# thrill/thrill

Measured on AMD Instinct MI355X. Metric: TeraSort keys/sec (100-byte recs), higher is better.
Workload: dtype u8; 1 GPU; terasort_10GiB_100B; records=107374182, record_bytes=100, seed=0x7421, parallelism=dp1

## Files before the change

### include/thrill_amd.h

```cpp
#ifndef THRILL_AMD_H
#define THRILL_AMD_H

#include <stdint.h>

#ifdef __cplusplus
extern "C" {
#endif

typedef struct t9_context t9_context;

int t9_create(t9_context** out, int device, int rank, int world, void* comm);
int t9_destroy(t9_context* ctx);
const char* t9_version(void);

int t9_comm_id_size(void);
int t9_comm_id(void* out_id);
int t9_comm_init(t9_context* ctx, const void* id);

int t9_gen_u64(t9_context* ctx, uint64_t* d_out, uint64_t index0, uint64_t n,
               uint64_t seed, void* stream);
int t9_gen_records(t9_context* ctx, uint8_t* d_out, uint64_t index0,
                   uint64_t n, uint64_t seed, void* stream);


// ... 18 lines not shown
                          uint32_t rec_size, int le, uint64_t* d_keys,
                          uint32_t* d_idx, uint32_t* d_hist, void* stream);

int t9_gather_records(t9_context* ctx, const uint8_t* d_recs,
                      const uint32_t* d_idx, uint64_t n, uint32_t rec_size,
                      uint8_t* d_out, void* stream);

uint64_t t9_sort_records_workspace(uint64_t n, uint32_t rec_size);
int t9_sort_records(t9_context* ctx, const uint8_t* d_in, uint8_t* d_out,
                    uint64_t n, uint32_t rec_size, uint32_t key_len,
                    void* d_workspace, void* stream);

int t9_sort_records_keyle(t9_context* ctx, const uint8_t* d_in,
                          uint8_t* d_out, uint64_t n, uint32_t rec_size,
                          void* d_workspace, void* stream);

int t9_sort_last_schedule(const t9_context* ctx);

int t9_sort_last_tiecount(const t9_context* ctx);

int t9_sort_last_fused(const t9_context* ctx);

int t9_sort_last_packed(const t9_context* ctx);


int t9_classify_u64(t9_context* ctx, const uint64_t* d_keys, uint64_t n,
                    uint64_t gidx0, const uint64_t* d_spl_keys,
                    const uint64_t* d_spl_idx, uint32_t p,
                    uint32_t* d_bucket, uint64_t* d_counts, void* stream);

int t9_classify_rec(t9_context* ctx, const uint8_t* d_recs,
                    const uint64_t* d_k64, uint64_t n, uint64_t gidx0,
                    const uint8_t* d_spl_recs, const uint64_t* d_spl_k64,
                    const uint64_t* d_spl_idx, uint32_t p, uint32_t rec_size,
                    uint32_t* d_bucket, uint64_t* d_counts, void* stream);

uint64_t t9_partition_idx_workspace(uint64_t n);
int t9_partition_idx(t9_context* ctx, const uint32_t* d_bucket, uint64_t n,
                     uint32_t p, uint32_t* d_perm, uint64_t* d_offsets,
                     void* d_workspace, void* stream);

int t9_alltoall(t9_context* ctx, const void* d_send,
                const uint64_t* send_counts, const uint64_t* send_displs,
                void* d_recv, const uint64_t* recv_counts,
                const uint64_t* recv_displs, uint64_t elem_size,
                void* stream);
// ... 148 lines not shown
```

### thrill_amd/csrc/t9_api.cpp

```cpp

#include "t9_common.h"

#include <rccl/rccl.h>

#include <cstdlib>
#include <cstring>
#include <new>

extern "C" {

const char* t9_version(void) { return "thrill_amd 0.1 (gfx950)"; }

int t9_create(t9_context** out, int device, int rank, int world,
              void* comm) {
    if (!out || world < 1 || rank < 0 || rank >= world) return T9_EINVAL;
    HIP_TRY(hipSetDevice(device));
    t9_context* ctx = new (std::nothrow) t9_context;
    if (!ctx) return T9_ENOMEM;
    ctx->device = device;
    ctx->rank = rank;
    ctx->world = world;
    ctx->comm = comm;
    ctx->owns_comm = 0;
    ctx->ov_stream = nullptr;
    for (int i = 0; i <= T9_OVERLAP_MAXK; ++i) ctx->ov_ev[i] = nullptr;
    ctx->ov_ready = 0;
    ctx->last_schedule = 0;
    ctx->last_tiecount = 0;
    ctx->last_fused = 0;
    ctx->last_packed = 0;
    *out = ctx;
    return T9_OK;
}

int t9_destroy(t9_context* ctx) {
    if (ctx && ctx->comm && ctx->owns_comm)
        ncclCommDestroy((ncclComm_t)ctx->comm);
    if (ctx) {
        if (ctx->ov_stream) {
            (void)hipStreamSynchronize(ctx->ov_stream);
            (void)hipStreamDestroy(ctx->ov_stream);
        }
        for (int i = 0; i <= T9_OVERLAP_MAXK; ++i)
            if (ctx->ov_ev[i]) (void)hipEventDestroy(ctx->ov_ev[i]);
    }
    delete ctx;
    return T9_OK;
}

int t9i_overlap_init(t9_context* ctx) {
    if (!ctx) return T9_EINVAL;
    if (ctx->ov_ready) return T9_OK;
    HIP_TRY(hipSetDevice(ctx->device));
// ... 2 lines not shown
                                         hipStreamNonBlocking));
    for (int i = 0; i <= T9_OVERLAP_MAXK; ++i)
        if (!ctx->ov_ev[i])
            HIP_TRY(hipEventCreateWithFlags(&ctx->ov_ev[i],
                                            hipEventDisableTiming));
    ctx->ov_ready = 1;
    return T9_OK;
}

int t9_sort_last_schedule(const t9_context* ctx) {
    return ctx ? ctx->last_schedule : T9_EINVAL;
}

int t9_sort_last_tiecount(const t9_context* ctx) {
    return ctx ? ctx->last_tiecount : T9_EINVAL;
}

int t9_sort_last_fused(const t9_context* ctx) {
    return ctx ? ctx->last_fused : T9_EINVAL;
}

int t9_sort_last_packed(const t9_context* ctx) {
    return ctx ? ctx->last_packed : T9_EINVAL;
}


int t9_comm_id_size(void) { return (int)sizeof(ncclUniqueId); }

int t9_comm_id(void* out_id) {
    if (!out_id) return T9_EINVAL;
    ncclResult_t rc = ncclGetUniqueId((ncclUniqueId*)out_id);
    if (rc != ncclSuccess) {
        fprintf(stderr, "t9_comm_id: %s\n", ncclGetErrorString(rc));
        return T9_EIO;
    }
    return T9_OK;
}

int t9_comm_init(t9_context* ctx, const void* id) {
    if (!ctx || !id) return T9_EINVAL;
    if (ctx->comm) return T9_EINVAL;
    HIP_TRY(hipSetDevice(ctx->device));
    ncclComm_t comm = nullptr;
    ncclResult_t rc = ncclCommInitRank(&comm, ctx->world,
                                       *(const ncclUniqueId*)id, ctx->rank);
    if (rc != ncclSuccess) {
// ... 68 lines not shown
```

### thrill_amd/csrc/t9_common.h

```cpp
#pragma once

#include <hip/hip_runtime.h>
#include <cstdint>
#include <cstdio>

#include "thrill_amd.h"

using u8 = uint8_t;
using u16 = uint16_t;
using u32 = uint32_t;
using u64 = uint64_t;

#define T9_WAVE 64

#define T9_OK 0
#define T9_EINVAL (-22)
#define T9_ENOMEM (-12)
#define T9_EIO (-5)
#define T9_ENOSYS (-38)

#define HIP_TRY(expr)                                                     \
    do {                                                                  \
        hipError_t _e = (expr);                                           \
        if (_e != hipSuccess) {                                           \
// ... 8 lines not shown
        hipError_t _e = hipGetLastError();                                \
        if (_e != hipSuccess) {                                           \
            fprintf(stderr, "t9: %s:%d: kernel launch failed: %s\n",      \
                    __FILE__, __LINE__, hipGetErrorString(_e));           \
            return T9_EIO;                                                \
        }                                                                 \
    } while (0)

#define T9_OVERLAP_MAXK 16

struct t9_context {
    int device;
    int rank;
    int world;
    void* comm;
    int owns_comm;
    hipStream_t ov_stream;
    hipEvent_t ov_ev[T9_OVERLAP_MAXK + 1];
    int ov_ready;
    int last_schedule;
    int last_tiecount;
    int last_fused;
    int last_packed;
};

#define T9_PK_IBITS 27
#define T9_PK_IMASK ((1u << T9_PK_IBITS) - 1u)

struct t9_overlap_req {
    const u8* recs;
    u8* out;
    u32 rec_words;
    u32 chunks;
    u32 fused;
    u32 keyle;
    u32 packed;
};

__host__ __device__ inline u64 t9_splitmix64_at(u64 seed, u64 ctr) {
    u64 z = seed + (ctr + 1) * 0x9E3779B97F4A7C15ull;
    z = (z ^ (z >> 30)) * 0xBF58476D1CE4E5B9ull;
    z = (z ^ (z >> 27)) * 0x94D049BB133111EBull;
    return z ^ (z >> 31);
}

__host__ __device__ inline u64 t9_hash128to64(u64 upper, u64 lower) {
    const u64 k = 0x9DDFEA08EB382D69ull;
    u64 a = (lower ^ upper) * k;
    a ^= (a >> 47);
    u64 b = (upper ^ a) * k;
    b ^= (b >> 47);
    b *= k;
    return b;
}

#define T9_MSB 0x8000000000000000ull

__host__ __device__ inline u64 t9_enc(u64 b, int op, int vtype) {
    if (op == T9_OP_SUM || vtype == T9_VAL_U64) return b;
// ... 28 lines not shown
```

### thrill_amd/csrc/t9_rank_scatter.h

```cpp
#pragma once
#include "t9_common.h"

template <int NDIG>
__device__ inline void t9_scan_onewave(u32* s_vals, u32 tid) {
    if (tid < 64) {
        const u32 lane = tid;
        u32 carry = 0;
        for (int c = 0; c < NDIG / 64; ++c) {
            const u32 v0 = s_vals[c * 64 + lane];
            u32 v = v0;
            for (int off = 1; off < 64; off <<= 1) {
                u32 y = __shfl_up(v, off);
                if (lane >= (u32)off) v += y;
            }
            const u32 total = __shfl(v, 63);
            s_vals[c * 64 + lane] = (v - v0) + carry;
            carry += total;
        }
    }
}

__device__ inline void t9_scan256_onewave(u32* s_vals, u32 tid) {
    if (tid < 64) {
        const u32 lane = tid;
// ... 162 lines not shown
            gpos[c] = s_goff[d] + (j - s_start[d]);
            out_keys[gpos[c]] = k;
        }
    }
    if (!HAS_VAL) return;
    __syncthreads();

#pragma unroll
    for (int g = 0; g < GROUPS; ++g) {
        const u32 i = wbase + g * 64 + lane;
        if (i < tn) {
            const u32 pos = (pos2[g >> 1] >> (16 * (g & 1))) & 0xffffu;
            if constexpr (LOAD_VAL) s_ovals[pos] = val[g];
            else s_ovals[pos] = (u32)(base + i);
        }
    }
    __syncthreads();
#pragma unroll
    for (int c = 0; c < GROUPS; ++c) {
        const u32 j = c * BLOCK + tid;
        if (j < tn) out_vals[gpos[c]] = s_ovals[j];
    }
}
```

### thrill_amd/csrc/t9_records.hip

```cpp

#include "t9_common.h"
#include "t9_rank_scatter.h"

#include <cstdlib>
#include <cstring>
#include <vector>
#include <algorithm>

extern "C" int t9i_sort_pairs_msb_unpacked_redo(u64*, u32*, u64, void*,
                                                void*, t9_overlap_req*,
                                                u32*);
extern "C" int t9i_count_tied(const u64* d_keys, u64 n, u32* d_ntied,
                              hipStream_t s);
extern "C" u64 t9_sort_pairs_workspace(u64 n);
extern "C" int t9_sort_pairs_u64_u32(t9_context*, u64*, u32*, u64, void*,
                                     void*);
extern "C" int t9i_sort_recs_msb(t9_context*, const u8*, u32, u64*, u32*,
                                 u64, void*, void*);
extern "C" u64 t9_partition_idx_workspace(u64 n);
extern "C" int t9_partition_idx(t9_context*, const u32*, u64, u32, u32*,
                                u64*, void*, void*);
extern "C" int t9i_sort_pairs_msb_ph(t9_context*, u64*, u32*, u64, void*,
                                     void*, int, t9_overlap_req*, u32*,
                                     int*);
// ... 783 lines not shown
        return T9_OK;
    }
    char* p = (char*)d_workspace;
    u64* d_keys = (u64*)p;
    p += t9_align256(n * 8);
    u32* d_idx = (u32*)p;
    p += t9_align256(n * 4);
    void* pair_ws = p;
    p += t9_sort_pairs_workspace(n);
    u32* d_ntied = (u32*)p;

    const char* algo = getenv("T9_SORT_ALGO");
    bool msb_dispatch = n >= (1ull << 22);
    if (algo && strcmp(algo, "lsd") == 0) msb_dispatch = false;
    if (algo && strcmp(algo, "msb") == 0) msb_dispatch = n >= (1ull << 14);
    const char* ehe = getenv("T9_EXTRACT_HIST");
    const u32 rw = rec_size / 4;
    const bool eh = !(ehe && ehe[0] == '0') && msb_dispatch &&
                    (rw == 25 || rw == 32);
    const char* fe = getenv("T9_FUSED_EXTRACT");
    bool fused = fe && atoi(fe) && n >= (1ull << 14) &&
                 (rec_size == 100 || rec_size == 128);
    int rc;
    t9_overlap_req ov = { nullptr, nullptr, 0, 0, 0, le ? 1u : 0u, 0 };
    int tie_counted = 0;
    if (ctx) {
        ctx->last_schedule = 0;
        ctx->last_tiecount = 0;
        ctx->last_fused = 0;
        ctx->last_packed = 0;
    }
    if (eh && !fused) {
        u32* hist = t9i_msb_pass1_hist(pair_ws, n);
        const u64 B = t9_ceil_div(n, 8192);
        const char* ie = getenv("T9_EXTRACT_IOTA");
        const bool widx = ie && ie[0] == '1';
        T9_PERF_WRAP(s, "extract",
                     launch_extract_hist_any(widx, rw, le, (u32)B, s, d_in,
                                             n, d_keys, d_idx, hist));
        T9_LAUNCH_CHECK();
        const char* gv = getenv("T9_GATHER_VARIANT");
        const bool may_overlap = rw == 25 && ctx && !(gv && atoi(gv) != 3);
        if (may_overlap) {
            ov.recs = d_in;
            ov.out = d_out;
            ov.rec_words = rw;
        }
        rc = t9i_sort_pairs_msb_ph(ctx, d_keys, d_idx, n, pair_ws, stream,
                                   widx ? 0 : 1, may_overlap ? &ov : nullptr,
                                   d_ntied, &tie_counted);
    }
    else if (fused && !le) {
        rc = t9i_sort_recs_msb(ctx, d_in, rec_size, d_keys, d_idx, n,
                               pair_ws, stream);
    }
    else {
        rc = le ? t9_extract_key64_le(ctx, d_in, n, rec_size, 0, d_keys,
                                      d_idx, stream)
                : t9_extract_key64(ctx, d_in, n, rec_size, 0, d_keys,
                                   d_idx, stream);
        if (rc) return rc;
        rc = t9_sort_pairs_u64_u32(ctx, d_keys, d_idx, n, pair_ws, stream);
    }
    if (rc) return rc;
    if (!tie_counted) {
        rc = t9i_count_tied(d_keys, n, d_ntied, s);
        if (rc) return rc;
    }
    if (ctx) ctx->last_tiecount = tie_counted;
    u32 ntied = 0;
    HIP_TRY(hipMemcpyAsync(&ntied, d_ntied, 4, hipMemcpyDeviceToHost, s));
    HIP_TRY(hipStreamSynchronize(s));
    if (ov.packed) {
        ctx->last_packed = ntied ? 2 : 1;
        if (ntied) {
            rc = t9i_sort_pairs_msb_unpacked_redo(d_keys, d_idx, n, pair_ws,
                                                  stream, &ov, d_ntied);
            if (rc) return rc;
            HIP_TRY(hipMemcpyAsync(&ntied, d_ntied, 4,
                                   hipMemcpyDeviceToHost, s));
            HIP_TRY(hipStreamSynchronize(s));
        }
    }
    if (ov.chunks) {
        ctx->last_schedule = (int)ov.chunks;
        if (!ntied) return T9_OK;
    }
    if (ov.fused) {
        ctx->last_fused = ntied ? 2 : 1;
        if (!ntied) return T9_OK;
    }

    if (ntied && rec_size > 8) {
        const u64 need = 6 * t9_align256(n * 4) +
                         2 * t9_align256(n * 8) +
                         t9_align256(3 * 8) + 256 +
                         t9_align256((n / T9_MAXSCAN_TILE + 2) * 4) + 256 +
                         t9_partition_idx_workspace(n);
        void* tmp_alloc = nullptr;
        char* q;
        if ((u64)n * rec_size >= need) {
            q = (char*)d_out;
        }
        else {
            HIP_TRY(hipMalloc(&tmp_alloc, need));
            q = (char*)tmp_alloc;
// ... 180 lines not shown
```

### thrill_amd/csrc/t9_sort_msb.hip

```cpp

#include "t9_common.h"
#include "t9_rank_scatter.h"
#include "t9_bitonic.h"

#include <cstdlib>
#include <vector>

#define T9_MSB_TILE 8192
#define T9_SUBMAX 4096
#define T9_MSB_MIN (1u << 22)

__global__ void k_colsum(const u32*, u64, u32*);
__global__ void k_chunkscan(u32*, u64, u32*);
__global__ void k_finaloffs(u32*, u64, const u32*, const u32*);
__global__ void k_grp_scan(u32*, u64, u64*);

extern "C" void t9i_launch_hist_seg9(u32, void*, const u64*, const u32*,
                                     const u32*, u32*);
extern "C" void t9i_launch_seg_scan9(u32, void*, u32*, const u32*,
                                     const u32*, const u32*, u32*, u32*);
extern "C" void t9i_launch_scatter_seg9(u32, int, void*, const u64*,
                                        const u32*, const u32*, const u32*,
                                        u64*, u32*, const u32*);
extern "C" void t9i_launch_scatter_seg9_packed(u32, void*, const u64*,
                                               const u32*, const u32*,
                                               const u32*, u64*, const u32*);
constexpr u64 NSUB9 = 256ull * 512;

static int pass2_bits() {
    const char* e = getenv("T9_PASS2_BITS");
    return (e && atoi(e) == 8) ? 8 : 9;
}

#define T9_L3_MIN 240000000ull

extern "C" int t9i_sort_pairs_lsd(t9_context*, u64*, u32*, u64, void*,
                                  void*);
extern "C" u64 t9i_sort_pairs_lsd_workspace(u64 n);
extern "C" int t9i_sort_keys_lsd(t9_context*, u64*, u64, void*, void*);


template <int RW>
__global__ __launch_bounds__(256) void k_hist_msb(
    const u64* __restrict__ keys, u64 n, u32 shift, u32* __restrict__ hist) {
    __shared__ u32 s_cnt[T9_RADIX];
    const u32 tid = threadIdx.x;
    const u64 base = (u64)blockIdx.x * T9_MSB_TILE;
    const u32 tn =
        (u32)((n - base < (u64)T9_MSB_TILE) ? (n - base) : (u64)T9_MSB_TILE);
// ... 908 lines not shown
#endif
#ifndef T9_FUSED_DEFAULT
#define T9_FUSED_DEFAULT 1
#endif

static bool t9i_fused_gather() {
    const char* e = getenv("T9_SORT_FUSED_GATHER");
    if (!e || e[0] == '\0') return T9_FUSED_DEFAULT != 0;
    return e[0] != '0';
}

static bool t9i_packed_ok(u64 n) {
    const char* e = getenv("T9_SORT_PACKED");
    if (e && e[0] == '0') return false;
    u32 bits = T9_PK_IBITS;
    const char* b = getenv("T9_SORT_PACKED_IDXBITS");
    if (b && b[0]) {
        const int v = atoi(b);
        if (v >= 1 && v < (int)T9_PK_IBITS) bits = (u32)v;
    }
    return n <= (1ull << bits);
}

static void t9i_launch_fused_wide(hipStream_t s, u64* d_keys, u32* d_vals,
                                  const u32* sub_start, const u32* sub_n,
                                  u32* tcount, const t9_overlap_req* ov) {
    hipLaunchKernelGGL(
        (k_wave16_sort_gather<T9_FUSED_D, T9_FUSED_TIES != 0>),
        dim3((u32)NSUB9), dim3(64), 0, s, d_keys, d_vals, sub_start, sub_n,
        tcount, (const u32*)ov->recs, (u32*)ov->out);
}

__global__ __launch_bounds__(64) void k_chunk_bounds(
    const u32* __restrict__ sub_start, u32 nsub, u32 K,
    const u32* __restrict__ info, u32* __restrict__ out) {
    const u32 c = threadIdx.x;
    if (c < 2) out[c] = info[c];
    if (c >= 1 && c < K)
        out[1 + c] = sub_start[(u64)c * nsub / K];
}

template <bool HAS_VAL, int RW = 0>
static int sort_msb_impl(t9_context* ctx, const u64* pass1_src,
                         u64* d_keys, u32* d_vals, u64 n,
                         void* d_workspace, void* stream,
                         bool pre_hist = false,
                         t9_overlap_req* ov = nullptr,
                         bool iota_vals = false,
                         u32* d_ntied = nullptr,
                         int* tie_counted = nullptr) {
    hipStream_t s = (hipStream_t)stream;
    MsbWs w = carve_msb((char*)d_workspace, n);

    {
        const u64 B = w.B1;
        const u64 Bc = t9_ceil_div(B, T9_SCAN_CHUNK);
        if (!pre_hist)
            T9_PERF_WRAP(s, "hist_pairs",
                         hipLaunchKernelGGL((k_hist_msb<RW>), dim3((u32)B),
                                            dim3(256), 0, s, pass1_src, n,
                                            56, w.hist));
        hipLaunchKernelGGL(k_colsum, dim3((u32)Bc), dim3(256), 0, s, w.hist,
                           B, w.chunkpart);
        hipLaunchKernelGGL(k_chunkscan, dim3(1), dim3(256), 0, s,
                           w.chunkpart, Bc, w.digit_base);
        hipLaunchKernelGGL(k_align_bases, dim3(1), dim3(256), 0, s,
                           w.digit_base, n, w.true_base, w.abase,
                           w.bucket_n);
        hipLaunchKernelGGL(k_finaloffs, dim3((u32)Bc), dim3(256), 0, s,
                           w.hist, B, w.chunkpart, w.abase);
        T9_PERF_WRAP(
            s, "pair_scatter",
            if (HAS_VAL && !RW && iota_vals)
                hipLaunchKernelGGL(
                    (k_scatter_wave512<T9_MSB_TILE, 1024, true, HAS_VAL, 0,
                                       true>),
                    dim3((u32)B), dim3(1024), 0, s, pass1_src, d_vals,
                    w.alt_k, w.alt_v, w.hist, n, 56);
            else
                hipLaunchKernelGGL(
                    (k_scatter_wave512<T9_MSB_TILE, 1024, true, HAS_VAL,
                                       RW>),
                    dim3((u32)B), dim3(1024), 0, s, pass1_src, d_vals,
                    w.alt_k, w.alt_v, w.hist, n, 56));
        T9_LAUNCH_CHECK();
    }

    {
        const char* l3x = getenv("T9_MSB_LEVELS");
        const bool blocked3 = (n >= T9_L3_MIN) ||
                              (l3x && atoi(l3x) == 3 && n >= (1ull << 14));
        if (pass2_bits() == 9 && !blocked3) {
            const u64 B2 = t9_ceil_div(n, T9_MSB_TILE) + 256;
            T9_PERF_WRAP(s, "hist_pairs",
                         t9i_launch_hist_seg9((u32)B2, stream, w.alt_k,
                                              w.abase, w.bucket_n,
                                              w.hist));
            t9i_launch_seg_scan9(256, stream, w.hist, w.abase, w.bucket_n,
                                 w.true_base, w.sub_start, w.sub_n);
            HIP_TRY(hipMemsetAsync(w.ovr, 0, 8, s));
            hipLaunchKernelGGL(k_subinfo, dim3((u32)(NSUB9 / 256)),
                               dim3(256), 0, s, w.sub_n, (u32)NSUB9,
                               T9_SUBMAX, NSUB, w.ovr, w.ovr + 2);
            const u32 K = (HAS_VAL && ov && ctx && !t9perf_on() &&
                           t9i_lds_wave16())
                              ? overlap_chunks() : 0;
            u32 info[2 + T9_OVERLAP_MAXK] = { 0, 0 };
            if (K) {
                hipLaunchKernelGGL(k_chunk_bounds, dim3(1), dim3(64), 0, s,
                                   w.sub_start, (u32)NSUB9, K, w.ovr,
                                   w.span);
                HIP_TRY(hipMemcpyAsync(info, w.span, (K + 1) * 4,
                                       hipMemcpyDeviceToHost, s));
            }
            else
                HIP_TRY(hipMemcpyAsync(info, w.ovr, 8,
                                       hipMemcpyDeviceToHost, s));
            HIP_TRY(hipStreamSynchronize(s));
            const u32 maxsub = info[0], novr9 = info[1];
            u32* tcount = nullptr;
            if constexpr (HAS_VAL) {
                if (d_ntied && novr9 == 0 &&
                    t9i_lds_wave16() && maxsub <= t9i_wave16_max()) {
                    tcount = d_ntied;
                    HIP_TRY(hipMemsetAsync(tcount, 0, 4, s));
                    if (tie_counted) *tie_counted = 1;
                }
            }
            bool fuse = false, packed = false;
            if constexpr (HAS_VAL) {
                fuse = tcount && ov && ctx && !t9perf_on() && ov->recs &&
                       ov->rec_words == 25 && overlap_chunks() == 0 &&
                       maxsub <= 1024 && t9i_fused_gather();
                packed = fuse && t9i_packed_ok(n);
            }
            if (packed)
                t9i_launch_scatter_seg9_packed((u32)B2, stream, w.alt_k,
                                               w.alt_v, w.abase, w.bucket_n,
                                               d_keys, w.hist);
            else
                T9_PERF_WRAP(s, "pair_scatter",
                             t9i_launch_scatter_seg9((u32)B2, HAS_VAL,
                                                     stream, w.alt_k,
                                                     w.alt_v, w.abase,
                                                     w.bucket_n, d_keys,
                                                     d_vals, w.hist));
            T9_LAUNCH_CHECK();
            if (K && tcount) {
                u64 bnd[T9_OVERLAP_MAXK + 1];
                bnd[0] = 0;
                bnd[K] = n;
                bool mono = true;
                for (u32 c = 1; c < K; ++c) {
                    bnd[c] = info[1 + c];
                    mono = mono && bnd[c] >= bnd[c - 1] && bnd[c] <= n;
                }
                if (mono) {
                    int rc = t9i_overlap_init(ctx);
                    if (rc) return rc;
// ... 19 lines not shown
                    }
                    HIP_TRY(hipEventRecord(ctx->ov_ev[T9_OVERLAP_MAXK], sb));
                    HIP_TRY(hipStreamWaitEvent(
                        s, ctx->ov_ev[T9_OVERLAP_MAXK], 0));
                    ov->chunks = done;
                    return T9_OK;
                }
            }
            if constexpr (HAS_VAL) {
                if (fuse) {
                    if (packed)
                        hipLaunchKernelGGL(
                            (k_wave16_sort_gather_packed<T9_FUSED_D>),
                            dim3((u32)NSUB9), dim3(64), 0, s, d_keys,
                            w.sub_start, w.sub_n, tcount,
                            (const u32*)ov->recs, (u32*)ov->out, ov->keyle,
                            (u32)(n - 1));
                    else
                        t9i_launch_fused_wide(s, d_keys, d_vals, w.sub_start,
                                              w.sub_n, tcount, ov);
                    T9_LAUNCH_CHECK();
                    ov->fused = 1;
                    ov->packed = packed ? 1 : 0;
                    return T9_OK;
                }
            }
            T9_PERF_WRAP(
                s, "lds_sort",
                if (t9i_lds_wave16() && maxsub <= t9i_wave16_max())
                    t9i_launch_wave16_sub<HAS_VAL>((u32)NSUB9, maxsub, s,
                                                   d_keys, d_vals,
                                                   w.sub_start, w.sub_n,
                                                   tcount);
                else if (t9i_lds_bitonic())
                    t9i_launch_bitonic_sub<HAS_VAL>((u32)NSUB9, maxsub, s,
                                                    d_keys, d_vals,
                                                    w.sub_start, w.sub_n);
                else if (maxsub <= 1024)
                    hipLaunchKernelGGL(
                        (k_lds_sort_sub<1024, 256, HAS_VAL>), dim3(NSUB9),
                        dim3(256), 0, s, d_keys, d_vals, w.sub_start,
                        w.sub_n);
                else if (maxsub <= 2048)
                    hipLaunchKernelGGL(
                        (k_lds_sort_sub<2048, 512, HAS_VAL>), dim3(NSUB9),
                        dim3(512), 0, s, d_keys, d_vals, w.sub_start,
// ... 322 lines not shown
```

### thrill_amd/csrc/t9_sort_msb9.hip

```cpp

#include "t9_common.h"
#include "t9_rank_scatter.h"

#include <cstdlib>
#include <vector>

#define T9_MSB_TILE 8192
#define NDIG9 512

__device__ inline u32 bucket_of9(const u32* s_abase, u32 pos) {
    u32 lo = 0, hi = 255;
    while (lo < hi) {
        u32 mid = (lo + hi + 1) >> 1;
        if (s_abase[mid] <= pos) lo = mid; else hi = mid - 1;
    }
    return lo;
}

__global__ __launch_bounds__(256) void k_hist_seg9(
    const u64* __restrict__ keys, const u32* __restrict__ abase,
    const u32* __restrict__ bucket_n, u32* __restrict__ hist) {
    __shared__ u32 s_cnt[NDIG9];
    __shared__ u32 s_abase[257];
    const u32 tid = threadIdx.x;
    s_abase[tid] = abase[tid];
    if (tid == 0) s_abase[256] = abase[256];
    s_cnt[tid] = 0;
    s_cnt[tid + 256] = 0;
    __syncthreads();
    const u64 tbase64 = (u64)blockIdx.x * T9_MSB_TILE;
    if (tbase64 < s_abase[256]) {
        const u32 tbase = (u32)tbase64;
        const u32 b = bucket_of9(s_abase, tbase);
        const u32 off = tbase - s_abase[b];
        const u32 tn = (bucket_n[b] > off)
                           ? ((bucket_n[b] - off < T9_MSB_TILE)
                                  ? bucket_n[b] - off
                                  : T9_MSB_TILE)
                           : 0;
        const u32 lane = tid & 63;
        for (u32 i0 = 0; i0 < (u32)T9_MSB_TILE; i0 += 256) {
            const u32 i = i0 + tid;
            const bool valid = i < tn;
            const u32 d =
                valid ? (u32)(keys[tbase + i] >> 47) & 511u : 0;
            t9_hist_ballot_add<9>(s_cnt, d, valid, lane);
        }
    }
    __syncthreads();
    hist[(u64)blockIdx.x * NDIG9 + tid] = s_cnt[tid];
    hist[(u64)blockIdx.x * NDIG9 + tid + 256] = s_cnt[tid + 256];
}

__global__ __launch_bounds__(256) void k_seg_scan9(
    u32* __restrict__ hist, const u32* __restrict__ abase,
    const u32* __restrict__ bucket_n, const u32* __restrict__ true_base,
    u32* __restrict__ sub_start, u32* __restrict__ sub_n) {
    const u32 b = blockIdx.x;
    const u32 tid = threadIdx.x;
    const u32 r0 = abase[b] / T9_MSB_TILE;
    const u32 rows = (bucket_n[b] + T9_MSB_TILE - 1) / T9_MSB_TILE;
    u32 tot0 = 0, tot1 = 0;
    for (u32 r = 0; r < rows; ++r) {
        tot0 += hist[(u64)(r0 + r) * NDIG9 + tid];
        tot1 += hist[(u64)(r0 + r) * NDIG9 + tid + 256];
    }
    __shared__ u32 sh[NDIG9];
    sh[tid] = tot0;
// ... 167 lines not shown
#pragma unroll
        for (int g = 0; g < GROUPS; ++g) {
            const u32 i = wbase + g * 64 + lane;
            if (i < tn)
                s_ovals[(pos2[g >> 1] >> (16 * (g & 1))) & 0xffffu] = val[g];
        }
        __builtin_amdgcn_sched_barrier(0);
    }
#pragma unroll
    for (int c = 0; c < GROUPS; ++c)
        if (c * 1024 + tid < tn) out_keys[gpos[c]] = k[c];
    if (!HAS_VAL) return;
    __syncthreads();
    {
        u32 v[GROUPS];
#pragma unroll
        for (int c = 0; c < GROUPS; ++c) v[c] = s_ovals[c * 1024 + tid];
#pragma unroll
        for (int c = 0; c < GROUPS; ++c)
            if (c * 1024 + tid < tn) out_vals[gpos[c]] = v[c];
    }
}

__global__ __launch_bounds__(1024, 8) void k_scatter_seg9_packed(
    const u64* __restrict__ in_keys, const u32* __restrict__ in_vals,
    const u32* __restrict__ abase, const u32* __restrict__ bucket_n,
    u64* __restrict__ out_comp, const u32* __restrict__ offs) {
    constexpr int TILE = T9_MSB_TILE;
    constexpr int NW = 16;
    constexpr int SUB = TILE / NW;
    constexpr int GROUPS = SUB / 64;
    __shared__ __align__(16) u8 s_raw[TILE * 8];
    u64* const s_ocomp = (u64*)s_raw;
    static_assert(SUB <= 65535 && TILE <= 65535, "u16 counts and offsets");
    static_assert(NW * 64 == 1024 && NDIG9 == 8 * 64,
                  "one thread per key column, waves 0..7 own the digits");
    __shared__ __align__(16) u16 s_wcnt[NW * NDIG9];
    u32* const s_wtot = (u32*)s_raw;
    u32* const s_delta = (u32*)s_wcnt;
    u8* const s_dig8 = (u8*)s_wcnt + NDIG9 * 4;
    u32* const s_hi = (u32*)((u8*)s_wcnt + NDIG9 * 4 + TILE);
    static_assert(NDIG9 * 4 + TILE + 4 <= NW * NDIG9 * 2,
                  "the overlays fit the count array");

    const u32 tid = threadIdx.x, wave = tid >> 6, lane = tid & 63;
    const u32 xper = gridDim.x >> 3, xrem = gridDim.x & 7;
    const u32 xcd = blockIdx.x & 7;
    const u32 tile = xcd * xper + (xcd < xrem ? xcd : xrem) +
                     (blockIdx.x >> 3);
    const u64 tbase64 = (u64)tile * TILE;
    if (tbase64 >= abase[256]) return;
    const u32 tbase = (u32)tbase64;

    const u32 wbase = wave * SUB;
    u64 key[GROUPS];
#pragma unroll
    for (int g = 0; g < GROUPS; ++g)
        key[g] = in_keys[tbase + wbase + g * 64 + lane];
    u32 val[GROUPS];
#pragma unroll
    for (int g = 0; g < GROUPS; ++g)
        val[g] = in_vals[tbase + wbase + g * 64 + lane];
    u32 ab[4], bnq[4];
#pragma unroll
    for (int q = 0; q < 4; ++q) {
        ab[q] = abase[q * 64 + lane];
        bnq[q] = bucket_n[q * 64 + lane];
    }
    u16* const wc = s_wcnt + wave * NDIG9;
    for (u32 t = lane; t < NDIG9; t += 64) wc[t] = 0;

    u32 nle = 0;
#pragma unroll
    for (int q = 0; q < 4; ++q)
        nle += (u32)__popcll(__ballot(ab[q] <= tbase));
    const u32 b = nle - 1, bq = b >> 6;
    const u32 ab_b = (u32)__builtin_amdgcn_readlane(
        (int)(bq == 0 ? ab[0] : bq == 1 ? ab[1] : bq == 2 ? ab[2] : ab[3]),
        (int)(b & 63));
    const u32 bn = (u32)__builtin_amdgcn_readlane(
        (int)(bq == 0 ? bnq[0] : bq == 1 ? bnq[1] : bq == 2 ? bnq[2]
                                                            : bnq[3]),
        (int)(b & 63));
    const u32 off_in_bucket = tbase - ab_b;
    const u32 tn = (bn > off_in_bucket)
                       ? ((bn - off_in_bucket < (u32)TILE)
                              ? bn - off_in_bucket
                              : (u32)TILE)
                       : 0;
    if (tn == 0) return;

    u32 pos2[GROUPS / 2] = {};
    u32 dig2[GROUPS / 2] = {};
#pragma unroll
    for (int g = 0; g < GROUPS; ++g) {
        const u32 i = wbase + g * 64 + lane;
        const bool valid = i < tn;
        const u32 d = (u32)(key[g] >> 47) & 511u;
        u32 dlo = 0, dhi = 0;
#pragma unroll
        for (int bit = 0; bit < 9; ++bit) {
            const u32 own = 0u - ((d >> bit) & 1u);
            const u64 bb = __ballot(own != 0);
            dlo |= (u32)bb ^ own;
            dhi |= (u32)(bb >> 32) ^ own;
        }
        const u64 m = __ballot(valid) & ~(((u64)dhi << 32) | dlo);
        const u32 wr = (u32)__popcll(m & ((1ull << lane) - 1ull));
        const u32 before = wc[d];
        pos2[g >> 1] |= (before + wr) << (16 * (g & 1));
        dig2[g >> 1] |= d << (16 * (g & 1));
        if (valid && wr == 0) wc[d] = (u16)(before + (u32)__popcll(m));
        key[g] = (((key[g] << 17) >> T9_PK_IBITS) << T9_PK_IBITS) |
                 (u64)val[g];
        asm volatile("" : "+v"(key[g]));
    }
#pragma unroll
    for (int q = 0; q < GROUPS / 2; ++q)
        asm volatile("" : "+v"(dig2[q]), "+v"(pos2[q]));
    u32 goff = 0;
    if (tid < NDIG9) goff = offs[(u64)tile * NDIG9 + tid];
    __syncthreads();

    u32 excl = 0;
    if (tid < NDIG9) {
        u32 run = 0;
        for (int w = 0; w < NW; ++w) {
            const u32 c = s_wcnt[w * NDIG9 + tid];
            s_wcnt[w * NDIG9 + tid] = (u16)run;
            run += c;
        }
        u32 v = run;
        for (int off = 1; off < 64; off <<= 1) {
            const u32 y = __shfl_up(v, off);
            if (lane >= (u32)off) v += y;
        }
        excl = v - run;
// ... 33 lines not shown

    const u32 hi = *s_hi;
    u64 k[GROUPS];
    u32 gpos[GROUPS];
#pragma unroll
    for (int c = 0; c < GROUPS; ++c) k[c] = s_ocomp[c * 1024 + tid];
#pragma unroll
    for (int c = 0; c < GROUPS; ++c) {
        const u32 j = c * 1024 + tid;
        const u32 d = (u32)s_dig8[j] | (j >= hi ? 256u : 0u);
        gpos[c] = s_delta[d] + j;
    }
#pragma unroll
    for (int c = 0; c < GROUPS; ++c)
        if (c * 1024 + tid < tn) out_comp[gpos[c]] = k[c];
}

extern "C" {

void t9i_launch_scatter_seg9_packed(u32 grid, void* stream,
                                    const u64* in_keys, const u32* in_vals,
                                    const u32* abase, const u32* bucket_n,
                                    u64* out_comp, const u32* offs) {
    hipLaunchKernelGGL(k_scatter_seg9_packed, dim3(grid), dim3(1024), 0,
                       (hipStream_t)stream, in_keys, in_vals, abase,
                       bucket_n, out_comp, offs);
}

void t9i_launch_hist_seg9(u32 grid, void* stream, const u64* keys,
                          const u32* abase, const u32* bucket_n,
                          u32* hist) {
    hipLaunchKernelGGL(k_hist_seg9, dim3(grid), dim3(256), 0,
                       (hipStream_t)stream, keys, abase, bucket_n, hist);
}

void t9i_launch_seg_scan9(u32 grid, void* stream, u32* hist,
                          const u32* abase, const u32* bucket_n,
                          const u32* true_base, u32* sub_start,
                          u32* sub_n) {
    hipLaunchKernelGGL(k_seg_scan9, dim3(grid), dim3(256), 0,
                       (hipStream_t)stream, hist, abase, bucket_n,
                       true_base, sub_start, sub_n);
}

void t9i_launch_scatter_seg9(u32 grid, int has_val, void* stream,
                             const u64* in_keys, const u32* in_vals,
                             const u32* abase, const u32* bucket_n,
                             u64* out_keys, u32* out_vals,
                             const u32* offs) {
    if (has_val)
        hipLaunchKernelGGL((k_scatter_seg9<true>), dim3(grid), dim3(1024),
                           0, (hipStream_t)stream, in_keys, in_vals, abase,
                           bucket_n, out_keys, out_vals, offs);
    else
        hipLaunchKernelGGL((k_scatter_seg9<false>), dim3(grid), dim3(1024),
                           0, (hipStream_t)stream, in_keys, in_vals, abase,
// ... 5 lines not shown
```

### thrill_amd/native.py

```python
import ctypes
import os

HERE = os.path.dirname(os.path.abspath(__file__))
SO = os.path.join(HERE, "libt9.so")

u64 = ctypes.c_uint64
u32 = ctypes.c_uint32
i32 = ctypes.c_int
vp = ctypes.c_void_p


T9_OP_SUM, T9_OP_MIN, T9_OP_MAX = 0, 1, 2
T9_VAL_U64, T9_VAL_I64, T9_VAL_F64 = 0, 1, 2
T9_EINVAL = -22


class T9Error(RuntimeError):
    pass


def lib_path():
    return SO


# ... 10 lines not shown
_SIGS = {
    "t9_version": (ctypes.c_char_p, []),
    "t9_create": (i32, [ctypes.POINTER(vp), i32, i32, i32, vp]),
    "t9_destroy": (i32, [vp]),
    "t9_comm_id_size": (i32, []),
    "t9_comm_id": (i32, [vp]),
    "t9_comm_init": (i32, [vp, vp]),
    "t9_gen_u64": (i32, [vp, vp, u64, u64, u64, vp]),
    "t9_gen_records": (i32, [vp, vp, u64, u64, u64, vp]),
    "t9_sort_u64_workspace": (u64, [u64]),
    "t9_sort_u64": (i32, [vp, vp, u64, vp, vp]),
    "t9_sort_pairs_workspace": (u64, [u64]),
    "t9_sort_pairs_u64_u32": (i32, [vp, vp, vp, u64, vp, vp]),
    "t9_extract_key64": (i32, [vp, vp, u64, u32, u32, vp, vp, vp]),
    "t9_extract_key64_hist": (i32, [vp, vp, u64, u32, i32, vp, vp, vp, vp]),
    "t9_gather_records": (i32, [vp, vp, vp, u64, u32, vp, vp]),
    "t9_sort_records_workspace": (u64, [u64, u32]),
    "t9_sort_records": (i32, [vp, vp, vp, u64, u32, u32, vp, vp]),
    "t9_sort_records_keyle": (i32, [vp, vp, vp, u64, u32, vp, vp]),
    "t9_sort_last_schedule": (i32, [vp]),
    "t9_sort_last_tiecount": (i32, [vp]),
    "t9_sort_last_fused": (i32, [vp]),
    "t9_sort_last_packed": (i32, [vp]),
    "t9_extract_key64_le": (i32, [vp, vp, u64, u32, u32, vp, vp, vp]),
    "t9_classify_u64": (i32, [vp, vp, u64, u64, vp, vp, u32, vp, vp, vp]),
    "t9_classify_rec": (i32, [vp, vp, vp, u64, u64, vp, vp, vp, u32, u32,
                              vp, vp, vp]),
    "t9_partition_idx_workspace": (u64, [u64]),
    "t9_partition_idx": (i32, [vp, vp, u64, u32, vp, vp, vp, vp]),
    "t9_alltoall": (i32, [vp, vp, vp, vp, vp, vp, vp, u64, vp]),
    "t9_hash_bucket": (i32, [vp, vp, u64, u64, u32, vp, vp, vp]),
    "t9_reduce_by_index": (i32, [vp, vp, vp, u64, u64, u64, vp, vp, vp]),
    "t9_index_bucket": (i32, [vp, vp, u64, u64, u64, u32, vp, vp, vp, vp]),
    "t9_reduce_init": (i32, [vp, vp, u64, vp]),
    "t9_reduce_build": (i32, [vp, vp, vp, u64, vp, u64, u64, vp, vp]),
    "t9_reduce_drain": (i32, [vp, vp, u64, vp, vp, vp, vp]),
    "t9_reduce128_table_words": (u64, [u64]),
    "t9_reduce128_init": (i32, [vp, vp, u64, vp]),
    "t9_reduce128_build": (i32, [vp, vp, vp, vp, u64, vp, u64, u64, vp,
                                 vp]),
    "t9_reduce128_drain": (i32, [vp, vp, u64, vp, vp, vp, vp, vp]),
    "t9_reduce128_lookup": (i32, [vp, vp, vp, u64, vp, u64, u64, vp, vp]),
    "t9_hash2_of": (i32, [vp, vp, u64, vp, vp, vp]),
    "t9_reduce_init_op": (i32, [vp, vp, u64, i32, i32, vp]),
    "t9_reduce_build_op": (i32, [vp, vp, vp, u64, vp, u64, u64, i32, i32,
                                 vp, vp]),
# ... 79 lines not shown
        k = self._lib.t9_sort_last_schedule(self.ctx)
        if k < 0:
            raise T9Error(f"t9_sort_last_schedule failed rc={k}")
        return k

    def sort_last_tiecount(self):
        k = self._lib.t9_sort_last_tiecount(self.ctx)
        if k < 0:
            raise T9Error(f"t9_sort_last_tiecount failed rc={k}")
        return k

    def sort_last_fused(self):
        k = self._lib.t9_sort_last_fused(self.ctx)
        if k < 0:
            raise T9Error(f"t9_sort_last_fused failed rc={k}")
        return k

    def sort_last_packed(self):
        k = self._lib.t9_sort_last_packed(self.ctx)
        if k < 0:
            raise T9Error(f"t9_sort_last_packed failed rc={k}")
        return k

    def perf_enable(self, on):
        self._lib.t9_perf_enable(1 if on else 0)

    def perf_read(self, cls):
        ms = ctypes.c_double()
        n = u64()
        rc = self._lib.t9_perf_read(cls.encode(), ctypes.byref(ms),
                                    ctypes.byref(n))
        if rc != 0:
            raise T9Error(f"t9_perf_read failed rc={rc}")
        return ms.value, n.value

    def perf_reset(self):
        self._lib.t9_perf_reset()

    def ws(self, name, *args):
        return getattr(self._lib, f"t9_{name}_workspace")(*args)

    def reduce128_table_words(self, capacity):
        return self._lib.t9_reduce128_table_words(capacity)

    def scan_geometry(self):
        t, p = u32(), u32()
# ... 26 lines not shown
```

Baseline: 10.64 billion keys/s.

## Pack index into key during MSB pass-1 scatter to drop separate value stream

Adds a pass-1 scatter kernel that writes a compressed 64-bit word (the key shifted past the first digit, with the record index in the low bits) instead of scattering keys and a separate u32 index array. The pass-2 packed scatter gains a variant that reads this compressed form directly, and the pass-2 histogram shift is adjusted to match. This removes the value reads and writes in both passes, cutting memory traffic. If ties remain after the shortened key, it falls back to a full wide re-sort from extraction, which costs extra work in that case.

```diff
diff --git a/include/thrill_amd.h b/include/thrill_amd.h
--- a/include/thrill_amd.h
+++ b/include/thrill_amd.h
@@ -64,6 +64,8 @@
 int t9_sort_last_fused(const t9_context* ctx);
 
 int t9_sort_last_packed(const t9_context* ctx);
+
+int t9_sort_last_pass1(const t9_context* ctx);
 
 
 int t9_classify_u64(t9_context* ctx, const uint64_t* d_keys, uint64_t n,
diff --git a/thrill_amd/csrc/t9_api.cpp b/thrill_amd/csrc/t9_api.cpp
--- a/thrill_amd/csrc/t9_api.cpp
+++ b/thrill_amd/csrc/t9_api.cpp
@@ -29,6 +29,7 @@
     ctx->last_tiecount = 0;
     ctx->last_fused = 0;
     ctx->last_packed = 0;
+    ctx->last_pass1 = 0;
     *out = ctx;
     return T9_OK;
 }
@@ -77,6 +78,10 @@
 
 int t9_sort_last_packed(const t9_context* ctx) {
     return ctx ? ctx->last_packed : T9_EINVAL;
+}
+
+int t9_sort_last_pass1(const t9_context* ctx) {
+    return ctx ? ctx->last_pass1 : T9_EINVAL;
 }
 
 
diff --git a/thrill_amd/csrc/t9_common.h b/thrill_amd/csrc/t9_common.h
--- a/thrill_amd/csrc/t9_common.h
+++ b/thrill_amd/csrc/t9_common.h
@@ -54,6 +54,7 @@
     int last_tiecount;
     int last_fused;
     int last_packed;
+    int last_pass1;
 };
 
 #define T9_PK_IBITS 27
@@ -67,6 +68,8 @@
     u32 fused;
     u32 keyle;
     u32 packed;
+    u32 pass1;
+    u32 wide;
 };
 
 __host__ __device__ inline u64 t9_splitmix64_at(u64 seed, u64 ctr) {
diff --git a/thrill_amd/csrc/t9_rank_scatter.h b/thrill_amd/csrc/t9_rank_scatter.h
--- a/thrill_amd/csrc/t9_rank_scatter.h
+++ b/thrill_amd/csrc/t9_rank_scatter.h
@@ -208,3 +208,116 @@
         if (j < tn) out_vals[gpos[c]] = s_ovals[j];
     }
 }
+
+template <int TILE, int BLOCK>
+__global__ __launch_bounds__(BLOCK, 8) void k_scatter_wave512_c1(
+    const u64* __restrict__ in_keys, u64* __restrict__ out_comp,
+    const u32* __restrict__ offs, u64 n, u32 ib1) {
+    constexpr int NW = BLOCK / 64;
+    constexpr int SUB = TILE / NW;
+    constexpr int GROUPS = SUB / 64;
+    static_assert(TILE % BLOCK == 0 && SUB % 64 == 0, "whole groups");
+    static_assert(GROUPS % 4 == 0, "digits are kept four to a register");
+    static_assert(TILE <= 65535, "u16 counts and offsets");
+    __shared__ __align__(16) u8 s_raw[TILE * 8];
+    u64* const s_ocomp = (u64*)s_raw;
+    __shared__ __align__(16) u16 s_wcnt[NW * T9_RADIX];
+    u8* const s_dig8 = (u8*)s_wcnt;
+    static_assert(TILE <= NW * T9_RADIX * 2, "the digits fit the counts");
+    __shared__ u32 s_start[T9_RADIX];
+    __shared__ u32 s_goff[T9_RADIX];
+
+    const u32 tid = threadIdx.x, wave = tid >> 6, lane = tid & 63;
+    const u32 xper = gridDim.x >> 3, xrem = gridDim.x & 7;
+    const u32 xcd = blockIdx.x & 7;
+    const u32 tile = xcd * xper + (xcd < xrem ? xcd : xrem) +
+                     (blockIdx.x >> 3);
+    const u64 base = (u64)tile * TILE;
+    const u32 tn = (u32)((n - base < (u64)TILE) ? (n - base) : (u64)TILE);
+
+    const u32 wbase = wave * SUB;
+    u64 key[GROUPS];
+#pragma unroll
+    for (int g = 0; g < GROUPS; ++g) {
+        const u32 i = wbase + g * 64 + lane;
+        key[g] = in_keys[base + (i < tn ? i : tn - 1)];
+    }
+
+    if (tid < T9_RADIX)
+        s_goff[tid] = offs[(u64)tile * T9_RADIX + tid];
+    u16* const wc = s_wcnt + wave * T9_RADIX;
+    for (u32 t = lane; t < T9_RADIX; t += 64) wc[t] = 0;
+
+    u32 pos2[GROUPS / 2] = {};
+    u32 dig4[GROUPS / 4] = {};
+#pragma unroll
+    for (int g = 0; g < GROUPS; ++g) {
+        const u32 i = wbase + g * 64 + lane;
+        const bool valid = i < tn;
+        const u32 d = (u32)(key[g] >> 56);
+        u64 m = __ballot(valid);
+        for (int bit = 0; bit < 8; ++bit) {
+            u64 bb = __ballot((d >> bit) & 1u);
+            m &= ((d >> bit) & 1u) ? bb : ~bb;
+        }
+        const u32 wr = (u32)__popcll(m & ((1ull << lane) - 1ull));
+        const u32 before = valid ? (u32)wc[d] : 0;
+        pos2[g >> 1] |= (before + wr) << (16 * (g & 1));
+        dig4[g >> 2] |= d << (8 * (g & 3));
+        if (valid && wr == 0) wc[d] = (u16)(before + (u32)__popcll(m));
+    }
+#pragma unroll
+    for (int g = 0; g < GROUPS; ++g) {
+        const u32 i = wbase + g * 64 + lane;
+        key[g] = (((key[g] << 8) >> ib1) << ib1) | (u64)((u32)base + i);
+        asm volatile("" : "+v"(key[g]));
+    }
+#pragma unroll
+    for (int q = 0; q < GROUPS / 2; ++q) asm volatile("" : "+v"(pos2[q]));
+#pragma unroll
+    for (int q = 0; q < GROUPS / 4; ++q) asm volatile("" : "+v"(dig4[q]));
+    __syncthreads();
+
+    if (tid < T9_RADIX) {
+        u32 run = 0;
+        for (int w = 0; w < NW; ++w) {
+            const u32 c = s_wcnt[w * T9_RADIX + tid];
+            s_wcnt[w * T9_RADIX + tid] = (u16)run;
+            run += c;
+        }
+        s_start[tid] = run;
+    }
+    __syncthreads();
+    t9_scan256_onewave(s_start, tid);
+    __syncthreads();
+
+#pragma unroll
+    for (int g = 0; g < GROUPS; ++g) {
+        const u32 i = wbase + g * 64 + lane;
+        if (i < tn) {
+            const u32 d = (dig4[g >> 2] >> (8 * (g & 3))) & 255u;
+            const u32 add = s_start[d] + (u32)wc[d];
+            const u32 pos = ((pos2[g >> 1] >> (16 * (g & 1))) & 0xffffu) + add;
+            s_ocomp[pos] = key[g];
+            pos2[g >> 1] += add << (16 * (g & 1));
+        }
+    }
+    __syncthreads();
+#pragma unroll
+    for (int g = 0; g < GROUPS; ++g) {
+        const u32 i = wbase + g * 64 + lane;
+        if (i < tn)
+            s_dig8[(pos2[g >> 1] >> (16 * (g & 1))) & 0xffffu] =
+                (u8)(dig4[g >> 2] >> (8 * (g & 3)));
+    }
+    __syncthreads();
+
+#pragma unroll
+    for (int c = 0; c < GROUPS; ++c) {
+        const u32 j = c * BLOCK + tid;
+        if (j < tn) {
+            const u32 d = s_dig8[j];
+            out_comp[s_goff[d] + (j - s_start[d])] = s_ocomp[j];
+        }
+    }
+}
diff --git a/thrill_amd/csrc/t9_records.hip b/thrill_amd/csrc/t9_records.hip
--- a/thrill_amd/csrc/t9_records.hip
+++ b/thrill_amd/csrc/t9_records.hip
@@ -829,13 +829,14 @@
     bool fused = fe && atoi(fe) && n >= (1ull << 14) &&
                  (rec_size == 100 || rec_size == 128);
     int rc;
-    t9_overlap_req ov = { nullptr, nullptr, 0, 0, 0, le ? 1u : 0u, 0 };
+    t9_overlap_req ov = { nullptr, nullptr, 0, 0, 0, le ? 1u : 0u, 0, 0, 0 };
     int tie_counted = 0;
     if (ctx) {
         ctx->last_schedule = 0;
         ctx->last_tiecount = 0;
         ctx->last_fused = 0;
         ctx->last_packed = 0;
+        ctx->last_pass1 = 0;
     }
     if (eh && !fused) {
         u32* hist = t9i_msb_pass1_hist(pair_ws, n);
@@ -874,21 +875,40 @@
         rc = t9i_count_tied(d_keys, n, d_ntied, s);
         if (rc) return rc;
     }
-    if (ctx) ctx->last_tiecount = tie_counted;
     u32 ntied = 0;
     HIP_TRY(hipMemcpyAsync(&ntied, d_ntied, 4, hipMemcpyDeviceToHost, s));
     HIP_TRY(hipStreamSynchronize(s));
+    if (ctx) ctx->last_pass1 = (int)ov.pass1;
     if (ov.packed) {
         ctx->last_packed = ntied ? 2 : 1;
-        if (ntied) {
+        if (ntied && ov.pass1) {
+            ctx->last_pass1 = 2;
+            ov.wide = 1;
+            ov.chunks = ov.fused = ov.packed = ov.pass1 = 0;
+            launch_extract_hist_any(false, rw, le, (u32)t9_ceil_div(n, 8192),
+                                    s, d_in, n, d_keys, d_idx,
+                                    t9i_msb_pass1_hist(pair_ws, n));
+            T9_LAUNCH_CHECK();
+            rc = t9i_sort_pairs_msb_ph(ctx, d_keys, d_idx, n, pair_ws, stream,
+                                       1, &ov, d_ntied, &tie_counted);
+            if (rc) return rc;
+            if (!tie_counted) {
+                rc = t9i_count_tied(d_keys, n, d_ntied, s);
+                if (rc) return rc;
+            }
+        }
+        else if (ntied) {
             rc = t9i_sort_pairs_msb_unpacked_redo(d_keys, d_idx, n, pair_ws,
                                                   stream, &ov, d_ntied);
             if (rc) return rc;
+        }
+        if (ntied) {
             HIP_TRY(hipMemcpyAsync(&ntied, d_ntied, 4,
                                    hipMemcpyDeviceToHost, s));
             HIP_TRY(hipStreamSynchronize(s));
         }
     }
+    if (ctx) ctx->last_tiecount = tie_counted;
     if (ov.chunks) {
         ctx->last_schedule = (int)ov.chunks;
         if (!ntied) return T9_OK;
diff --git a/thrill_amd/csrc/t9_sort_msb.hip b/thrill_amd/csrc/t9_sort_msb.hip
--- a/thrill_amd/csrc/t9_sort_msb.hip
+++ b/thrill_amd/csrc/t9_sort_msb.hip
@@ -16,7 +16,7 @@
 __global__ void k_grp_scan(u32*, u64, u64*);
 
 extern "C" void t9i_launch_hist_seg9(u32, void*, const u64*, const u32*,
-                                     const u32*, u32*);
+                                     const u32*, u32*, u32);
 extern "C" void t9i_launch_seg_scan9(u32, void*, u32*, const u32*,
                                      const u32*, const u32*, u32*, u32*);
 extern "C" void t9i_launch_scatter_seg9(u32, int, void*, const u64*,
@@ -25,6 +25,11 @@
 extern "C" void t9i_launch_scatter_seg9_packed(u32, void*, const u64*,
                                                const u32*, const u32*,
                                                const u32*, u64*, const u32*);
+extern "C" void t9i_launch_scatter_seg9_packed_c1(u32, void*, const u64*,
+                                                  const u32*, const u32*,
+                                                  u64*, const u32*, u32);
+extern "C" void t9i_launch_scatter_pass1_c1(u32, void*, const u64*, u64*,
+                                            const u32*, u64, u32);
 constexpr u64 NSUB9 = 256ull * 512;
 
 static int pass2_bits() {
@@ -979,6 +984,27 @@
     return n <= (1ull << bits);
 }
 
+#ifndef T9_PACKED1_DEFAULT
+#define T9_PACKED1_DEFAULT 1
+#endif
+static bool t9i_packed1_on() {
+    const char* e = getenv("T9_SORT_PACKED1");
+    if (!e || e[0] == '\0') return T9_PACKED1_DEFAULT != 0;
+    return e[0] != '0';
+}
+
+static u32 t9i_packed1_ib(u64 n) {
+    u32 ib = 1;
+    while (ib < T9_PK_IBITS && ((n - 1) >> ib)) ++ib;
+    const char* b = getenv("T9_SORT_PACKED1_IDXBITS");
+    if (b && b[0]) {
+        int v = atoi(b);
+        if (v > (int)T9_PK_IBITS) v = T9_PK_IBITS;
+        if (v > (int)ib) ib = (u32)v;
+    }
+    return ib;
+}
+
 static void t9i_launch_fused_wide(hipStream_t s, u64* d_keys, u32* d_vals,
                                   const u32* sub_start, const u32* sub_n,
                                   u32* tcount, const t9_overlap_req* ov) {
@@ -1008,6 +1034,20 @@
                          int* tie_counted = nullptr) {
     hipStream_t s = (hipStream_t)stream;
     MsbWs w = carve_msb((char*)d_workspace, n);
+
+    bool c1 = false;
+    u32 ib1 = 0;
+    if constexpr (HAS_VAL && RW == 0) {
+        const char* l3c = getenv("T9_MSB_LEVELS");
+        const bool l3 = (n >= T9_L3_MIN) ||
+                        (l3c && atoi(l3c) == 3 && n >= (1ull << 14));
+        c1 = pre_hist && iota_vals && d_ntied && ov && !ov->wide && ctx &&
+             !t9perf_on() && ov->recs && ov->rec_words == 25 &&
+             overlap_chunks() == 0 && t9i_fused_gather() &&
+             t9i_lds_wave16() && pass2_bits() == 9 && !l3 &&
+             t9i_packed_ok(n) && t9i_packed1_on();
+        if (c1) ib1 = t9i_packed1_ib(n);
+    }
 
     {
         const u64 B = w.B1;
@@ -1028,7 +1068,10 @@
                            w.hist, B, w.chunkpart, w.abase);
         T9_PERF_WRAP(
             s, "pair_scatter",
-            if (HAS_VAL && !RW && iota_vals)
+            if (c1)
+                t9i_launch_scatter_pass1_c1((u32)B, stream, pass1_src,
+                                            w.alt_k, w.hist, n, ib1);
+            else if (HAS_VAL && !RW && iota_vals)
                 hipLaunchKernelGGL(
                     (k_scatter_wave512<T9_MSB_TILE, 1024, true, HAS_VAL, 0,
                                        true>),
@@ -1052,7 +1095,7 @@
             T9_PERF_WRAP(s, "hist_pairs",
                          t9i_launch_hist_seg9((u32)B2, stream, w.alt_k,
                                               w.abase, w.bucket_n,
-                                              w.hist));
+                                              w.hist, c1 ? 55u : 47u));
             t9i_launch_seg_scan9(256, stream, w.hist, w.abase, w.bucket_n,
                                  w.true_base, w.sub_start, w.sub_n);
             HIP_TRY(hipMemsetAsync(w.ovr, 0, 8, s));
@@ -1089,9 +1132,22 @@
                 fuse = tcount && ov && ctx && !t9perf_on() && ov->recs &&
                        ov->rec_words == 25 && overlap_chunks() == 0 &&
                        maxsub <= 1024 && t9i_fused_gather();
-                packed = fuse && t9i_packed_ok(n);
-            }
-            if (packed)
+                packed = fuse && !ov->wide && t9i_packed_ok(n);
+            }
+            if (c1 && !packed) {
+                ov->wide = 1;
+                if (tie_counted) *tie_counted = 0;
+                const int rc = sort_msb_impl<HAS_VAL, RW>(
+                    ctx, pass1_src, d_keys, d_vals, n, d_workspace, stream,
+                    false, ov, iota_vals, d_ntied, tie_counted);
+                ov->pass1 = 2;
+                return rc;
+            }
+            if (packed && c1)
+                t9i_launch_scatter_seg9_packed_c1((u32)B2, stream, w.alt_k,
+                                                  w.abase, w.bucket_n,
+                                                  d_keys, w.hist, ib1);
+            else if (packed)
                 t9i_launch_scatter_seg9_packed((u32)B2, stream, w.alt_k,
                                                w.alt_v, w.abase, w.bucket_n,
                                                d_keys, w.hist);
@@ -1157,6 +1213,7 @@
                     T9_LAUNCH_CHECK();
                     ov->fused = 1;
                     ov->packed = packed ? 1 : 0;
+                    ov->pass1 = (packed && c1) ? 1 : 0;
                     return T9_OK;
                 }
             }
diff --git a/thrill_amd/csrc/t9_sort_msb9.hip b/thrill_amd/csrc/t9_sort_msb9.hip
--- a/thrill_amd/csrc/t9_sort_msb9.hip
+++ b/thrill_amd/csrc/t9_sort_msb9.hip
@@ -19,7 +19,7 @@
 
 __global__ __launch_bounds__(256) void k_hist_seg9(
     const u64* __restrict__ keys, const u32* __restrict__ abase,
-    const u32* __restrict__ bucket_n, u32* __restrict__ hist) {
+    const u32* __restrict__ bucket_n, u32* __restrict__ hist, u32 shift) {
     __shared__ u32 s_cnt[NDIG9];
     __shared__ u32 s_abase[257];
     const u32 tid = threadIdx.x;
@@ -43,7 +43,7 @@
             const u32 i = i0 + tid;
             const bool valid = i < tn;
             const u32 d =
-                valid ? (u32)(keys[tbase + i] >> 47) & 511u : 0;
+                valid ? (u32)(keys[tbase + i] >> shift) & 511u : 0;
             t9_hist_ballot_add<9>(s_cnt, d, valid, lane);
         }
     }
@@ -257,10 +257,11 @@
     }
 }
 
+template <bool C1IN>
 __global__ __launch_bounds__(1024, 8) void k_scatter_seg9_packed(
     const u64* __restrict__ in_keys, const u32* __restrict__ in_vals,
     const u32* __restrict__ abase, const u32* __restrict__ bucket_n,
-    u64* __restrict__ out_comp, const u32* __restrict__ offs) {
+    u64* __restrict__ out_comp, const u32* __restrict__ offs, u32 ib1) {
     constexpr int TILE = T9_MSB_TILE;
     constexpr int NW = 16;
     constexpr int SUB = TILE / NW;
@@ -292,10 +293,14 @@
 #pragma unroll
     for (int g = 0; g < GROUPS; ++g)
         key[g] = in_keys[tbase + wbase + g * 64 + lane];
-    u32 val[GROUPS];
-#pragma unroll
-    for (int g = 0; g < GROUPS; ++g)
-        val[g] = in_vals[tbase + wbase + g * 64 + lane];
+    u32 val[C1IN ? 1 : GROUPS];
+    if constexpr (!C1IN) {
+#pragma unroll
+        for (int g = 0; g < GROUPS; ++g)
+            val[g] = in_vals[tbase + wbase + g * 64 + lane];
+    }
+    const u32 csh = (ib1 + 9 > T9_PK_IBITS) ? ib1 + 9 : (u32)T9_PK_IBITS;
+    const u64 imask1 = (1ull << ib1) - 1ull;
     u32 ab[4], bnq[4];
 #pragma unroll
     for (int q = 0; q < 4; ++q) {
@@ -331,7 +336,8 @@
     for (int g = 0; g < GROUPS; ++g) {
         const u32 i = wbase + g * 64 + lane;
         const bool valid = i < tn;
-        const u32 d = (u32)(key[g] >> 47) & 511u;
+        const u32 d = C1IN ? (u32)(key[g] >> 55)
+                           : (u32)(key[g] >> 47) & 511u;
         u32 dlo = 0, dhi = 0;
 #pragma unroll
         for (int bit = 0; bit < 9; ++bit) {
@@ -346,8 +352,11 @@
         pos2[g >> 1] |= (before + wr) << (16 * (g & 1));
         dig2[g >> 1] |= d << (16 * (g & 1));
         if (valid && wr == 0) wc[d] = (u16)(before + (u32)__popcll(m));
-        key[g] = (((key[g] << 17) >> T9_PK_IBITS) << T9_PK_IBITS) |
-                 (u64)val[g];
+        if constexpr (C1IN)
+            key[g] = (((key[g] << 9) >> csh) << csh) | (key[g] & imask1);
+        else
+            key[g] = (((key[g] << 17) >> T9_PK_IBITS) << T9_PK_IBITS) |
+                     (u64)val[g];
         asm volatile("" : "+v"(key[g]));
     }
 #pragma unroll
@@ -427,16 +436,35 @@
                                     const u64* in_keys, const u32* in_vals,
                                     const u32* abase, const u32* bucket_n,
                                     u64* out_comp, const u32* offs) {
-    hipLaunchKernelGGL(k_scatter_seg9_packed, dim3(grid), dim3(1024), 0,
-                       (hipStream_t)stream, in_keys, in_vals, abase,
-                       bucket_n, out_comp, offs);
+    hipLaunchKernelGGL((k_scatter_seg9_packed<false>), dim3(grid),
+                       dim3(1024), 0, (hipStream_t)stream, in_keys, in_vals,
+                       abase, bucket_n, out_comp, offs, 0u);
+}
+
+void t9i_launch_scatter_seg9_packed_c1(u32 grid, void* stream,
+                                       const u64* in_comp, const u32* abase,
+                                       const u32* bucket_n, u64* out_comp,
+                                       const u32* offs, u32 ib1) {
+    hipLaunchKernelGGL((k_scatter_seg9_packed<true>), dim3(grid),
+                       dim3(1024), 0, (hipStream_t)stream, in_comp,
+                       (const u32*)nullptr, abase, bucket_n, out_comp, offs,
+                       ib1);
+}
+
+void t9i_launch_scatter_pass1_c1(u32 grid, void* stream, const u64* in_keys,
+                                 u64* out_comp, const u32* offs, u64 n,
+                                 u32 ib1) {
+    hipLaunchKernelGGL((k_scatter_wave512_c1<T9_MSB_TILE, 1024>), dim3(grid),
+                       dim3(1024), 0, (hipStream_t)stream, in_keys, out_comp,
+                       offs, n, ib1);
 }
 
 void t9i_launch_hist_seg9(u32 grid, void* stream, const u64* keys,
                           const u32* abase, const u32* bucket_n,
-                          u32* hist) {
+                          u32* hist, u32 shift) {
     hipLaunchKernelGGL(k_hist_seg9, dim3(grid), dim3(256), 0,
-                       (hipStream_t)stream, keys, abase, bucket_n, hist);
+                       (hipStream_t)stream, keys, abase, bucket_n, hist,
+                       shift);
 }
 
 void t9i_launch_seg_scan9(u32 grid, void* stream, u32* hist,
diff --git a/thrill_amd/native.py b/thrill_amd/native.py
--- a/thrill_amd/native.py
+++ b/thrill_amd/native.py
@@ -56,6 +56,7 @@
     "t9_sort_last_tiecount": (i32, [vp]),
     "t9_sort_last_fused": (i32, [vp]),
     "t9_sort_last_packed": (i32, [vp]),
+    "t9_sort_last_pass1": (i32, [vp]),
     "t9_extract_key64_le": (i32, [vp, vp, u64, u32, u32, vp, vp, vp]),
     "t9_classify_u64": (i32, [vp, vp, u64, u64, vp, vp, u32, vp, vp, vp]),
     "t9_classify_rec": (i32, [vp, vp, vp, u64, u64, vp, vp, vp, u32, u32,
@@ -181,6 +182,12 @@
             raise T9Error(f"t9_sort_last_packed failed rc={k}")
         return k
 
+    def sort_last_pass1(self):
+        k = self._lib.t9_sort_last_pass1(self.ctx)
+        if k < 0:
+            raise T9Error(f"t9_sort_last_pass1 failed rc={k}")
+        return k
+
     def perf_enable(self, on):
         self._lib.t9_perf_enable(1 if on else 0)
 
```

Result: no change. 10.72 billion keys/s (median of 6 runs) (+0.7%).
